# Zachary-Luk/3D-Denoising-Diffusion-Model

Hardware: AMD Instinct MI355X
Metric: denoised 64³ volumes/sec @250 DDPM steps, 1/2/4/8 MI355X; PSNR vs ref (higher is better)
Workload: dtype f32 (conv products: 3x f16-split MFMA, f32 accumulate)

## Files before the change

3d-denoising-diffusion-model_amd/csrc/api.hip:

```cpp
#include <hip/hip_runtime.h>
#include <stdarg.h>
#include <stdio.h>
#include <string.h>
#include "conv3d_params.h"
#include "ddpm3d.h"
#include "ops.h"
#include "noise.h"

static thread_local char g_err[512] = "";

static int fail(int code, const char* fmt, ...) {
    va_list ap;
    va_start(ap, fmt);
    vsnprintf(g_err, sizeof(g_err), fmt, ap);
    va_end(ap);
    return code;
}
static int launched(hipError_t e, const char* what) {
    if (e == hipSuccess) return DDPM3D_OK;
    return fail(DDPM3D_ELAUNCH, "%s: %s", what, hipGetErrorString(e));
}

extern "C" {

// ... 188 lines not shown
        route = ddpm3d_pw_ok(k, c, d->ksize) ? ROUTE_PW : ROUTE_GENERAL;
    return DDPM3D_OK;
}

int ddpm3d_conv3d(const ddpm3d_conv_desc* d, void* stream) {
    ConvK k;
    ConvCfg c;
    int route = ROUTE_GENERAL;
    const int ok = conv_prepare(d, k, c, route, true);
    if (ok != DDPM3D_OK) return ok;
    if (route == ROUTE_SKINNY)
        return launched(ddpm3d_launch_conv_skinny(k, d->precision, (hipStream_t)stream), "conv3d (skinny)");
    const int rc = route == ROUTE_PW ? launched(ddpm3d_launch_conv_pw(k, c, (hipStream_t)stream), "conv3d (1x1)")
                                     : launched(ddpm3d_launch_conv(k, c, (hipStream_t)stream), "conv3d");
    if (rc != DDPM3D_OK || c.S == 1) return rc;
    return launched(ddpm3d_launch_splitk_reduce(k, (hipStream_t)stream), "conv3d split-K reduce");
}

static int base_prec(int p) {
    return p == DDPM3D_PREC_F16X3_WZ ? DDPM3D_PREC_F16X3 : p == DDPM3D_PREC_F16_WZ ? DDPM3D_PREC_F16
         : p == DDPM3D_PREC_BF16_WZ ? DDPM3D_PREC_BF16 : p;
}
static int skip_prepare(const ddpm3d_conv_desc* d, const ddpm3d_conv_skip* sk, ddpm3d_conv_desc& sd, ConvK& k, ConvCfg& c,
                        bool& fused, bool for_launch) {
    fused = false;
    if (!d || !sk) return fail(DDPM3D_EINVAL, "conv3d_skip: null descriptor");
    if (d->res_mode != DDPM3D_RES_NONE || d->res)
        return fail(DDPM3D_EINVAL, "conv3d_skip: conv2 carries no residual of its own (the skip conv is its residual)");
    if (d->out_layout != DDPM3D_OUT_NDHWC) return fail(DDPM3D_EINVAL, "conv3d_skip: NDHWC output only");
    if (d->ksize != 3) return fail(DDPM3D_EINVAL, "conv3d_skip: conv2 is a 3x3x3 conv (ksize %d)", d->ksize);
// ... 32 lines not shown
    k.sk_bound = sk->in_bound; k.sk_bound_count = sk->in_bound_count; k.sk_bound_stride = sk->in_bound_stride;
    k.sk_blocks_per_split = (sd.Cin / 32 + c.S - 1) / c.S;
    return DDPM3D_OK;
}

int ddpm3d_conv3d_skip(const ddpm3d_conv_desc* d, const ddpm3d_conv_skip* sk, void* stream) {
    ddpm3d_conv_desc sd;
    ConvK k;
    ConvCfg c;
    bool fused = false;
    const int ok = skip_prepare(d, sk, sd, k, c, fused, true);
    if (ok != DDPM3D_OK) return ok;
    if (fused) {
        const int rc = launched(ddpm3d_launch_conv(k, c, (hipStream_t)stream), "conv3d_skip");
        if (rc != DDPM3D_OK || c.S == 1) return rc;
        return launched(ddpm3d_launch_splitk_reduce(k, (hipStream_t)stream), "conv3d_skip split-K reduce");
    }
    const int rc = ddpm3d_conv3d(&sd, stream);
    if (rc != DDPM3D_OK) return rc;
    ddpm3d_conv_desc d2 = *d;
    d2.res = d->out;
    d2.res_mode = DDPM3D_RES_SAME;
    if (d->io_dtype & DDPM3D_IO_OUT_BF16) d2.io_dtype |= DDPM3D_IO_RES_BF16;
    return ddpm3d_conv3d(&d2, stream);
}

int ddpm3d_conv_skip_fused(const ddpm3d_conv_desc* d, const ddpm3d_conv_skip* sk) {
    ddpm3d_conv_desc sd;
    ConvK k;
    ConvCfg c;
// ... 1017 lines not shown
```

3d-denoising-diffusion-model_amd/csrc/conv3d.hip:

```cpp
#include <hip/hip_runtime.h>
#include "conv3d_load.h"
#include "conv3d_epilogue.h"

template <int PREC, int PIPEM, int KS, int WN, int MT, int TXL, int TYL>
__global__ __launch_bounds__(256, (PIPEM == 2 ? 1 : (TXL == 2 ? 2 : 3))) void conv3d_kernel(const ConvK p) {
    constexpr int CK = DDPM3D_CONV_CK;
    constexpr int PIPE = PIPEM == 1 ? 1 : 0;
    constexpr int SXY = PIPEM == 2 ? 2 : 1;
    constexpr int WM = 4 / WN;
    constexpr int TX = 1 << TXL, TY = 1 << TYL;
    constexpr int TZ = WM * MT * 32 / (TX * TY);
    constexpr int PAD = KS / 2;
    constexpr int HX = SXY * (TX - 1) + KS, HY = SXY * (TY - 1) + KS, HZ = TZ + 2 * PAD;
    constexpr int HV = HX * HY * HZ;
    constexpr int VS = 5;
    constexpr int RY = LdsGeom<TX, HX, HY>::RY;
    constexpr int RZ = LdsGeom<TX, HX, HY>::RZ;
    constexpr int QPV = CK / 4;
    constexpr int NT = KS * KS * KS;
    constexpr int NL = (HV * QPV + 255) / 256;

    extern __shared__ __attribute__((aligned(16))) unsigned char lds[];

    const int tid = threadIdx.x;
// ... 367 lines not shown

#if DDPM3D_PREC_ONLY == 3
#include "conv3d_wz.h"
#ifndef DDPM3D_WZ_T84
#define DDPM3D_WZ_T84 1
#endif
hipError_t ddpm3d_launch_conv_wz(const ConvK& k, const ConvCfg& c, hipStream_t st) {
    const int gy = k.CoutPad / 128;
    const int gx = k.N * k.tilesZ * k.tilesY * k.tilesX;
#ifdef DDPM3D_WZ_STAMPS
    constexpr size_t stamp_lds = 4 * WZ_NSTAMP * 8;
#else
    constexpr size_t stamp_lds = 0;
#endif
    constexpr size_t lds = (size_t)WzGeom::BUF + stamp_lds;
    if (k.sk_w != nullptr) {
        if (c.PREC != DDPM3D_PREC_F16X3_WZ) return hipErrorInvalidValue;
        constexpr size_t slds4 = (size_t)WzGeomT<4>::BUF + stamp_lds, slds84 = (size_t)WzGeomT<8, 4>::BUF + stamp_lds;
        if (c.TXL == 2)
            hipLaunchKernelGGL((conv3d_wz_kernel<WZ_F16X3_SKIP, 4, 4>), dim3(gx, gy, k.ksplit), dim3(256), slds4, st, k);
        else if (DDPM3D_WZ_T84 && k.H % 8 == 0 && k.D % 4 == 0) {
            ConvK k2 = k;
            k2.tilesY = 2 * k.tilesY;
            k2.tilesZ = k.tilesZ / 2;
            hipLaunchKernelGGL((conv3d_wz_kernel<WZ_F16X3_SKIP, 4, 8, 4>), dim3(gx, gy, k.ksplit), dim3(256), slds84, st, k2);
        } else
            hipLaunchKernelGGL((conv3d_wz_kernel<WZ_F16X3_SKIP, 4>), dim3(gx, gy, k.ksplit), dim3(256), lds, st, k);
        return hipGetLastError();
    }
    if (k.hint & DDPM3D_HINT_UP_PHASE) {
// ... 96 lines not shown
```

3d-denoising-diffusion-model_amd/csrc/conv3d_params.h:

```cpp
#pragma once
#include <hip/hip_runtime.h>
#include <stddef.h>
#include <stdlib.h>
#include "ddpm3d.h"

#define DDPM3D_CONV_CK 16
#define DDPM3D_REDUCE_VOX 16
#define DDPM3D_X3_W_TARGET 8.0f

struct ConvK {
    const float* src0;
    const float* src1;
    const float* affA;
    const float* affB;
    const float* w;
    const float* bias;
    const float* res;
    float* out;
    double* stats;
    float* partial;
    const float* wscale;
    const float* in_bound;
    int in_bound_count, in_bound_stride;
    unsigned w_bytes, src0_bytes, src1_bytes;
// ... 106 lines not shown
    }
    const long long vox = (long long)D * H * W;
    c.reduce_vox = DDPM3D_REDUCE_VOX;
    while (c.reduce_vox > 4 &&
           (long long)N * ((vox + c.reduce_vox - 1) / c.reduce_vox) * ((Cout / 4 + 63) / 64) < 1024)
        c.reduce_vox /= 2;
    ddpm3d_conv_cfg_split(c, best, N, D, H, W, Cout);
    return c;
}

static inline bool ddpm3d_skip_fuse_rule(int N, int D, int H, int W, int Cx, int Cout, const ConvCfg& c) {
    (void)N; (void)D; (void)H; (void)W; (void)Cx; (void)Cout; (void)c;
    return true;
}

static inline size_t ddpm3d_packed_bytes(int Cout, int Cin, int ksize, int prec) {
    const size_t taps = (prec == DDPM3D_PREC_F16X3_WZ || prec == DDPM3D_PREC_F16_WZ || prec == DDPM3D_PREC_BF16_WZ)
                            ? 36 : (size_t)ksize * ksize * ksize;
    const size_t body = taps * ddpm3d_cin_pad(Cin) * ddpm3d_cout_pad(Cout) * 4;
    return prec != 0 ? body + (size_t)ddpm3d_cout_pad(Cout) * 4 : body;
}

static inline size_t ddpm3d_up_phase_body_bytes(int Cout, int Cin) {
    return (size_t)64 * ddpm3d_cin_pad(Cin) * ddpm3d_cout_pad(Cout) * 4;
}
static inline size_t ddpm3d_up_phase_bytes(int Cout, int Cin) {
    return ddpm3d_packed_bytes(Cout, Cin, 3, DDPM3D_PREC_F16X3_WZ) + ddpm3d_up_phase_body_bytes(Cout, Cin) +
           (size_t)ddpm3d_cout_pad(Cout) * 4;
}
struct UpPhaseGeom { int TX, TY, tilesX, tilesY, tilesZ; };
// ... 101 lines not shown
```

3d-denoising-diffusion-model_amd/csrc/conv3d_stage.h:

```cpp
#pragma once
#include "conv3d_epilogue.h"

enum { WZ_F16X3 = 0, WZ_F16 = 1, WZ_BF16 = 2,
       WZ_F16X3_UP = 3,
       WZ_F16X3_SKIP = 4 };

__device__ __forceinline__ void split_pair(float s0, float s1, unsigned& hi, unsigned& lo) {
    float l0, l1;
    asm("v_cvt_pk_f16_f32 %0, %3, %4\n\t"
        "v_fma_mix_f32 %1, %0, -1.0, %3 op_sel:[0,0,0] op_sel_hi:[1,0,0]\n\t"
        "v_fma_mix_f32 %2, %0, -1.0, %4 op_sel:[1,0,0] op_sel_hi:[1,0,0]"
        : "=&v"(hi), "=&v"(l0), "=&v"(l1)
        : "v"(s0), "v"(s1));
    asm("v_cvt_pk_f16_f32 %0, %1, %2" : "=v"(lo) : "v"(l0), "v"(l1));
}

template <int TX_, int TY_ = TX_>
struct WzGeomT {
    static constexpr int CK = DDPM3D_CONV_CK;
    static constexpr int TX = TX_, TY = TY_, HX = TX_ + 2, HY = TY_ + 2, NP = 4, VS = 5;
    static constexpr int RP = TX_ * TY_;
    static constexpr int NZP = 64 / RP;
    static constexpr int NPL = 2 * NZP + 2;
    static constexpr int RY = LdsGeom<TX_, HX, HY>::RY;
// ... 179 lines not shown
```

3d-denoising-diffusion-model_amd/csrc/conv3d_wz.h:

```cpp
#pragma once
#include "conv3d_stage.h"

#ifdef DDPM3D_WZ_STAMPS
#define WZ_NSTAMP 48
#define WZ_STAMP(i) do { if (lane == 0) wz_stamps[(i)] = __builtin_amdgcn_s_memtime(); } while (0)
#else
#define WZ_STAMP(i) do { } while (0)
#endif

template <int MODE_, int IL = 0, int TX = 8, int TY = TX>
__global__ __launch_bounds__(256, 2) void conv3d_wz_kernel(const ConvK p) {
    constexpr bool PHASE = MODE_ == WZ_F16X3_UP;
    constexpr bool SKIP = MODE_ == WZ_F16X3_SKIP;
    constexpr int MODE = (PHASE || SKIP) ? (int)WZ_F16X3 : MODE_;
    typedef WzGeomT<TX, TY> G;
    constexpr bool X3 = MODE == WZ_F16X3;
    constexpr int CK = DDPM3D_CONV_CK, NT = PHASE ? 16 : 36;
    constexpr int TPJ = NT / 4;
    constexpr int TXL = TX == 8 ? 3 : 2, TYL = TY == 8 ? 3 : 2;
    constexpr int VS = G::VS, RY = G::RY, RZ = G::RZ;

    extern __shared__ __attribute__((aligned(16))) unsigned char lds[];

    const int tid = threadIdx.x;
    const int lane = tid & 63;
    const int wn = __builtin_amdgcn_readfirstlane(tid >> 6);
    const int half = lane >> 5;
#ifdef DDPM3D_WZ_STAMPS
    unsigned long long* wz_stamps = reinterpret_cast<unsigned long long*>(lds + G::BUF) + wn * WZ_NSTAMP;
    WZ_STAMP(0);
#endif

    const WgId wg = wg_id(p);
    int tile = wg.tile;
    const int tx_i = tile % p.tilesX; tile /= p.tilesX;
    const int ty_i = tile % p.tilesY; tile /= p.tilesY;
    const int tz_i = tile % p.tilesZ; tile /= p.tilesZ;
    const int ph = PHASE ? (tile & 3) : 0;
    const int py = ph >> 1, px = ph & 1;
    const int n = PHASE ? tile >> 2 : tile;
    const int x0 = tx_i * TX, y0 = ty_i * TY, z0 = tz_i * 2 * G::NZP;

    int arow[2];
#pragma unroll
    for (int t = 0; t < 2; ++t) {
        const int m = t * 32 + (lane & 31);
        const int pos = m % G::RP;
        arow[t] = (m / G::RP) * G::PAIR + ((pos >> TXL) * RY + (pos & (TX - 1)) * VS + half) * 16;
        if constexpr (PHASE) arow[t] += (py * RY + px * VS) * 16;
    }

    const int cout = wg.cy * 128 + wn * 32 + (lane & 31);
    const float pre_ws = cout < p.Cout ? p.wscale[cout] : 1.0f;
    const float pre_bias = cout < p.Cout ? p.bias[(size_t)n * p.bias_stride_n + cout] : 0.0f;
    const __amdgpu_buffer_rsrc_t wrsrc = make_rsrc(p.w, p.w_bytes);
    const unsigned wlane = ((unsigned)cout * 2 + half) * 16;
    const unsigned wpart = (unsigned)p.CoutPad * 32;
    const unsigned wchunk_stride = 2 * wpart;
    const unsigned wtap_stride = (unsigned)(p.CinPad / CK) * wchunk_stride;

    f32x16 acc[4][2];
#pragma unroll
    for (int j = 0; j < 4; ++j)
#pragma unroll
        for (int t = 0; t < 2; ++t)
#pragma unroll
            for (int i = 0; i < 16; ++i) acc[j][t][i] = 0.0f;

    const int nchunks = p.CinPad / CK;
    const int chunk_begin = wg.split * p.chunks_per_split;
    const int chunk_end = min(nchunks, chunk_begin + p.chunks_per_split);

    ActScale asc = {1.0f, 1.0f};
    float bound_raw = 0.0f;
    if constexpr (MODE != WZ_BF16) bound_raw = act_scale_load(p, n);
    float sk_bound_raw = 0.0f;
    ActScale ax = {1.0f, 1.0f};
    if constexpr (SKIP)
        if (lane < p.sk_bound_count) sk_bound_raw = p.sk_bound[((size_t)n * p.sk_bound_count + lane) * p.sk_bound_stride];
    StageLaneT<G> sl = stage_lane<G, PHASE>(p, tid, n, y0, x0, max(z0 - 1, 0), 1.0f);
    stage_zero_border(sl, lds, 1, tid);
    StageRawT<G> raw;
    if (chunk_begin < chunk_end) stage_issue(p, sl, raw, n, z0, chunk_begin);
    if constexpr (MODE != WZ_BF16) {
        asc = act_scale_finish(bound_raw, 2.0f);
        if constexpr (SKIP) ax = act_scale_finish(sk_bound_raw, 1.0f);
        stage_lane_scale(p, sl, asc.s);
    }
    WZ_STAMP(1);

    constexpr int L = X3 ? 1 : 0;
#ifndef DDPM3D_WZ_RING_X3
#define DDPM3D_WZ_RING_X3 4
#endif
#ifndef DDPM3D_WZ_RING_X1
// ... 92 lines not shown
#pragma unroll
                for (int i = 0; i < (X3 ? 2 : 1); ++i) {
                    __builtin_amdgcn_sched_group_barrier(0x008, 1, 0);
                    __builtin_amdgcn_sched_group_barrier(0x020, 1, 0);
                }
#pragma unroll
                for (int i = 0; i < (X3 ? 4 : 2); ++i) {
                    __builtin_amdgcn_sched_group_barrier(0x008, 1, 0);
                    __builtin_amdgcn_sched_group_barrier(0x100, 1, 0);
                }
            }
        }
        if constexpr (IL == 3 || IL == 4 || IL == 6) __builtin_amdgcn_s_setprio(0);
        WZ_STAMP(6 + (chunk - chunk_begin) * 5);
    }
    WZ_STAMP(42);

    f32x16 outv[4];
#pragma unroll
    for (int t = 0; t < 2; ++t) {
        outv[t] = acc[0][t] + acc[1][t] + acc[2][t];
        outv[2 + t] = acc[1][t] - acc[2][t] - acc[3][t];
    }
    const int tile_in_n = ((ph * p.tilesZ + tz_i) * p.tilesY + ty_i) * p.tilesX + tx_i;
    if constexpr (SKIP) {
        const int tid_ = tid;
        constexpr int XB = 32, XROW = VS * 16, XCH = 128 * XROW;
        static_assert(2 * XCH <= G::BUF, "an x block fits the tile's image");
        const int nxb = (p.sk_C0 + p.sk_C1) / XB;
        const int xb_begin = wg.split * p.sk_blocks_per_split;
        const int xb_end = min(nxb, xb_begin + p.sk_blocks_per_split);
        int tid = tid_;
        asm volatile("" : "+v"(tid));
        const int lane = tid & 63, half = lane >> 5;
        const int xq = tid & 7;
        unsigned xv0[4], xv1[4];
#pragma unroll
        for (int i = 0; i < 4; ++i) {
            const int m = (tid >> 3) + 32 * i;
            const int z = z0 + epi_tz<TXL, TYL, G::NZP != 1>(m), y = y0 + ((m >> TXL) & (TY - 1)), x = x0 + (m & (TX - 1));
            const bool inb = z < p.D && y < p.H && x < p.W;
            const unsigned vox = (unsigned)(((n * p.D + z) * p.H + y) * p.W + x);
            xv0[i] = inb ? (vox * (unsigned)p.sk_C0 + xq * 4u) * 4u : DDPM3D_OOB_OFFSET;
            xv1[i] = inb ? (vox * (unsigned)p.sk_C1 + xq * 4u) * 4u : DDPM3D_OOB_OFFSET;
        }
        const int xl = ((xq >> 2) * 128 + (tid >> 3)) * XROW + (xq & 3) * 8;
        const int xa = ((lane & 31) * VS + half) * 16;
        auto x_issue = [&](const int b, u32x4 (&xr)[4]) {
            const bool valid = b < xb_end;
            const int c0 = b * XB;
            const bool from0 = c0 < p.sk_C0;
            const __amdgpu_buffer_rsrc_t rs = make_rsrc(from0 ? p.sk_src0 : p.sk_src1,
                                                        valid ? (from0 ? p.sk_src0_bytes : p.sk_src1_bytes) : 0u);
            const unsigned soff = valid ? (unsigned)(from0 ? c0 : c0 - p.sk_C0) * 4u : 0u;
#pragma unroll
            for (int i = 0; i < 4; ++i) xr[i] = buffer_load16(rs, from0 ? xv0[i] : xv1[i], soff);
        };
        auto w_issue = [&](const int b, u32x4 (&wq)[2][2]) {
            const bool valid = b < xb_end;
            const __amdgpu_buffer_rsrc_t rs = make_rsrc(p.sk_w, valid ? p.sk_w_bytes : 0u);
            const unsigned soff = valid ? (unsigned)(2 * b) * wchunk_stride : 0u;
#pragma unroll
// ... 33 lines not shown
                const h8 bhi = __builtin_bit_cast(h8, wq[c][0]), blo = __builtin_bit_cast(h8, wq[c][1]);
#pragma unroll
                for (int u = 0; u < 4; ++u) {
                    const unsigned char* a = lds + c * XCH + u * 32 * XROW + xa;
                    const h8 ahi = *reinterpret_cast<const h8*>(a), alo = *reinterpret_cast<const h8*>(a + 32);
                    outv[u] = mfma16<false>(alo, bhi, outv[u]);
                    outv[u] = mfma16<false>(ahi, blo, outv[u]);
                    outv[u] = mfma16<false>(ahi, bhi, outv[u]);
                }
            }
        };
        for (int b = xb_begin; b < xb_end; b += 2) {
            x_block(b, xr, wa, wb);
            x_block(b + 1, xr, wb, wa);
        }
        const float bias2 = pre_bias + sk_bias;
        if (p.ksplit > 1)
            conv_epilogue<1, 1, 4, TXL, TYL, true, G::NZP != 1, true, false>(p, outv, n, z0, y0, x0, tile_in_n, 0, cout, half, wg.split,
                                                                     ax.inv, true, sk_ws, bias2, 0, 0);
        else
            conv_epilogue<1, 1, 4, TXL, TYL, false, G::NZP != 1, false, false>(p, outv, n, z0, y0, x0, tile_in_n, 0, cout, half, wg.split,
                                                                     ax.inv, true, sk_ws, bias2, 0, 0);
        return;
    }
    #ifndef DDPM3D_WZ_WIDE_X3
#define DDPM3D_WZ_WIDE_X3 0
#endif
#ifndef DDPM3D_WZ_LEAN
#define DDPM3D_WZ_LEAN 1
#endif
    constexpr bool LEAN = DDPM3D_WZ_LEAN && MODE != WZ_F16X3;
    const float ws1[1] = {pre_ws}, bs1[1] = {pre_bias};
    if (p.ksplit > 1) {
        if (LEAN && conv_epilogue_lean<1, 1, 4, 1, TXL, TYL, G::NZP != 1, true>(p, outv, n, z0, y0, x0, tile_in_n, 0, cout, half,
                                                                                         wg.split, asc.inv, ws1, bs1)) {
        } else
        conv_epilogue<1, 1, 4, TXL, TYL, true, G::NZP != 1, true, PHASE>(p, outv, n, z0, y0, x0, tile_in_n, 0, cout, half, wg.split,
                                                                 asc.inv, true, pre_ws, pre_bias, py, px);
    } else if (LEAN &&
               conv_epilogue_lean<1, 1, 4, 1, TXL, TYL, G::NZP != 1, false>(p, outv, n, z0, y0, x0, tile_in_n, 0, cout, half, wg.split,
                                                                           asc.inv, ws1, bs1)) {
    } else
    conv_epilogue<1, 1, 4, TXL, TYL, MODE != WZ_F16X3 || DDPM3D_WZ_WIDE_X3, G::NZP != 1, false, PHASE>(p, outv, n, z0, y0, x0, tile_in_n, 0, cout, half, wg.split,
                                                                 asc.inv, true, pre_ws, pre_bias, py, px);
#ifdef DDPM3D_WZ_STAMPS
    WZ_STAMP(43);
    if (lane == 0) {
        wz_stamps[44] = __builtin_amdgcn_s_getreg((31 << 11) | 4);
        wz_stamps[45] = __builtin_amdgcn_s_getreg((31 << 11) | 20);
        wz_stamps[46] = __builtin_amdgcn_s_memrealtime();
    }
    if (p.partial != nullptr && lane < WZ_NSTAMP) {
        const size_t wgl = blockIdx.x + (size_t)gridDim.x * (blockIdx.y + (size_t)gridDim.y * blockIdx.z);
        float* dump = p.partial + (p.ksplit > 1 ? (size_t)p.ksplit * p.N * p.D * p.H * p.W * p.Cout : (size_t)0);
        reinterpret_cast<unsigned long long*>(dump)[(wgl * 4 + wn) * WZ_NSTAMP + lane] = wz_stamps[lane];
    }
#endif
}
```

3d-denoising-diffusion-model_amd/csrc/unet_plan.hip:

```cpp
#include <hip/hip_runtime.h>
#include <stdarg.h>
#include <stdio.h>
#include <string.h>
#include <map>
#include <new>
#include <vector>
#include "ddpm3d.h"

namespace {

struct Act {
    size_t off = 0;
    int C = 0, D = 0, H = 0, W = 0;
    int esize = 4;
    size_t stats_off = 0;
    int rows = 0;
    size_t bytes(int N) const { return (size_t)N * D * H * W * C * esize; }
    long long voxels() const { return (long long)D * H * W; }
};

enum StepKind { S_CONV, S_FINALIZE, S_ABSMAX, S_PAD, S_POOL, S_ATTN };

struct Step {
    int kind;
// ... 87 lines not shown
        int act = DDPM3D_ACT_NONE, in_mode = DDPM3D_IN_SAME;
        const Act* res = nullptr; int res_mode = DDPM3D_RES_NONE;
        bool planar = false, want_stats = true, bias_per_n = false;
        bool ncdhw_out = false;
        size_t bound = 0; int bound_first = 0, bound_count = 0, bound_stride = 0; bool has_bound = false;
        int film_off = 0;
        const ddpm3d_conv_weights* skip_w = nullptr;
        const Act* x0 = nullptr; const Act* x1 = nullptr;
        size_t xbound = 0; int xbound_first = 0; bool has_xbound = false;
        bool* fused = nullptr;
    };
    bool conv_step(const ddpm3d_conv_weights& pc, ConvArgs a, int* step_index = nullptr) {
        ddpm3d_conv_desc d;
        memset(&d, 0, sizeof(d));
        const bool wz = pc.w_packed_wz && !a.planar && (a.in_mode == DDPM3D_IN_SAME || a.in_mode == DDPM3D_IN_UP);
        d.precision = wz ? (pc.precision_wz & ~DDPM3D_WZ_UP_PHASE_IMAGE) : (pc.precision & ~DDPM3D_SKIP_TWO_CALLS);
        d.w_packed = wz ? pc.w_packed_wz : pc.w_packed;
        if (wz && (pc.precision_wz & DDPM3D_WZ_UP_PHASE_IMAGE) && a.in_mode == DDPM3D_IN_UP)
            d.kernel_hint = DDPM3D_HINT_UP_PHASE;
        d.bias = pc.bias;
        d.Cout = pc.Cout; d.ksize = pc.ksize;
        const Act* geo = a.out ? a.out : a.src0;
        d.N = N; d.D = geo->D; d.H = geo->H; d.W = geo->W;
        d.out_layout = a.ncdhw_out ? DDPM3D_OUT_NCDHW : DDPM3D_OUT_NDHWC;
        if (a.planar) {
            d.in_mode = DDPM3D_IN_PLANAR2; d.Cin = 2; d.C0 = 1; d.C1 = 1;
        } else {
            d.in_mode = a.in_mode;
            d.src0 = (const float*)at(a.src0->off); d.C0 = a.src0->C;
            if (a.src1) { d.src1 = (const float*)at(a.src1->off); d.C1 = a.src1->C; }
            d.Cin = d.C0 + d.C1;
            if (d.Cin != pc.Cin) return fail("conv %dx%d fed %d channels", pc.Cout, pc.Cin, d.Cin);
            if (a.src0->esize == 2) d.io_dtype |= DDPM3D_IO_SRC0_BF16;
            if (a.src1 && a.src1->esize == 2) d.io_dtype |= DDPM3D_IO_SRC1_BF16;
// ... 370 lines not shown
```

3d-denoising-diffusion-model_amd/guided_diffusion/_hip.py:

```python

import ctypes as C
import os

import torch

_HERE = os.path.dirname(os.path.abspath(__file__))
LIB_PATH = os.environ.get("DDPM3D_LIB") or os.path.normpath(os.path.join(_HERE, "..", "csrc", "libddpm3d.so"))

IN_SAME, IN_POOL, IN_UP, IN_PLANAR2, IN_STRIDE2 = 0, 1, 2, 3, 4
RES_NONE, RES_SAME, RES_POOL, RES_UP = 0, 1, 2, 3
ACT_NONE, ACT_SILU = 0, 1
OUT_NDHWC, OUT_NCDHW = 0, 1
F_LEARN_SIGMA, F_PREDICT_XSTART, F_CLIP = 1, 2, 4
NCOEF = 8
NQCOEF = 4
NSCOEF = 8
S_CX, S_W0, S_W1, S_W2, S_CZ = 0, 1, 2, 3, 4
PREC_F32, PREC_F16X3, PREC_F16, PREC_F16X3_WZ, PREC_F16_WZ, PREC_BF16, PREC_BF16_WZ = 0, 1, 2, 3, 4, 5, 6
PRECISIONS = {"f32": PREC_F32, "f16x3": PREC_F16X3, "f16": PREC_F16, "bf16": PREC_BF16}
WINOGRAD_OF = {PREC_F16X3: PREC_F16X3_WZ, PREC_F16: PREC_F16_WZ, PREC_BF16: PREC_BF16_WZ}
IO_SRC0_BF16, IO_SRC1_BF16, IO_OUT_BF16, IO_RES_BF16 = 1, 2, 4, 8
IO_HALF_IS_F16 = 16
ABI_VERSION = 13
MAX_DRAWS = 64
MAX_QUANTILES = 8
HINT_WSTAT_OFF, HINT_WSTAT_ON = 0x100, 0x200
HINT_SPLITK_SHIFT = 16
HINT_WZ_ORDER_SHIFT = 12
HINT_UP_PHASE = 0x400
WZ_UP_PHASE_IMAGE = 0x100
SKIP_TWO_CALLS = 0x100

_fp = C.c_void_p


class ConvDesc(C.Structure):
    _fields_ = [
        ("N", C.c_int32), ("D", C.c_int32), ("H", C.c_int32), ("W", C.c_int32),
        ("Cin", C.c_int32), ("Cout", C.c_int32), ("ksize", C.c_int32), ("in_mode", C.c_int32),
        ("src0", _fp), ("src1", _fp), ("C0", C.c_int32), ("C1", C.c_int32),
        ("aff_a", _fp), ("aff_b", _fp), ("act", C.c_int32), ("precision", C.c_int32),
        ("w_packed", _fp), ("bias", _fp), ("bias_stride_n", C.c_int32), ("res_mode", C.c_int32),
        ("res", _fp), ("out", _fp), ("out_layout", C.c_int32), ("stats_rows", C.c_int32),
        ("stats", _fp), ("workspace", _fp), ("workspace_bytes", C.c_size_t),
# ... 251 lines not shown
```

3d-denoising-diffusion-model_amd/guided_diffusion/engine.py:

```python

import collections
import ctypes as C
import math
import os

import torch

from . import _hip as H


class Act:
    __slots__ = ("buf", "C", "D", "H", "W", "stats", "rows")

    def __init__(self, buf, Cn, D, Hh, W, stats, rows):
        self.buf, self.C, self.D, self.H, self.W, self.stats, self.rows = buf, Cn, D, Hh, W, stats, rows

    @property
    def half(self):
        return self.buf.dtype in (torch.bfloat16, torch.float16)

    @property
    def voxels(self):
        return self.D * self.H * self.W

# ... 58 lines not shown
        qkv_perm = {}
        if getattr(topo, "new_attention_order", False):
            for e in topo.all_layers():
                if e.kind == "attn":
                    Cn, ch = e.cin, e.cin // e.heads
                    leg = torch.arange(3 * Cn)
                    h, part, i = leg // (3 * ch), (leg // ch) % 3, leg % ch
                    qkv_perm[e.prefix + ".qkv"] = (part * Cn + h * ch + i).to(device)
        params = dict(params)
        for base, perm in qkv_perm.items():
            params[base + ".weight"] = params[base + ".weight"][perm].contiguous()
            params[base + ".bias"] = params[base + ".bias"][perm].contiguous()
        self.p = params
        self.up_phase = (winograd and precision == "f16x3" and os.environ.get("DDPM3D_UP_PHASE", "1") != "0")
        self.skip_fuse = os.environ.get("DDPM3D_SKIP_FUSE", "1") != "0"
        up_conv1 = {e.prefix + ".in_layers.2" for e in topo.all_layers() if e.kind == "res" and e.updown == "up"}
        for name, t in params.items():
            if name.endswith(".weight") and t.dim() >= 3:
                base = name[:-len(".weight")]
                if t.dim() == 5:
                    w = t
                elif t.dim() == 4 and t.shape[2] == 3:
                    w = torch.zeros(t.shape[0], t.shape[1], 3, 3, 3, dtype=t.dtype, device=t.device)
                    w[:, :, 1] = t
                else:
                    w = t.reshape(t.shape[0], t.shape[1], 1, 1, 1)
                if base == first and not planar and w.shape[1] != self.cin_pad:
                    wp = torch.zeros(w.shape[0], self.cin_pad, *w.shape[2:], dtype=w.dtype, device=w.device)
                    wp[:, :w.shape[1]] = w
                    w = wp
# ... 57 lines not shown
            pl = _Plan(self, N, D, Hh, W)
            self.plans[key] = pl
        else:
            self.plans.move_to_end(key)
        return pl

    def _conv_weights(self, pc):
        w = H.ConvWeights()
        if pc is not None:
            w.w_packed, w.bias = H.ptr(pc.w), H.ptr(pc.b)
            w.Cout, w.Cin, w.ksize, w.precision = pc.Cout, pc.Cin, pc.k, pc.precision
            if pc.wz is not None:
                w.w_packed_wz, w.precision_wz = H.ptr(pc.wz.w), pc.wz.precision
                if pc.wz.up_phase:
                    w.precision_wz |= H.WZ_UP_PHASE_IMAGE
        return w

    def native_desc(self):
        if self._native_desc is not None:
            return self._native_desc[0]
        topo, p = self.topo, self.p
        layers, keep = [], []

        def one(e):
            L = H.Layer()
            L.updown, L.heads = H.UPDOWN[e.updown], e.heads
            if e.kind == "res":
                L.kind = H.LAYER_RES
                L.film_off = self.film_off[e.prefix]
                L.norm1_gamma, L.norm1_beta = H.ptr(p[e.prefix + ".in_layers.0.weight"]), H.ptr(p[e.prefix + ".in_layers.0.bias"])
# ... 333 lines not shown
            io |= H.IO_SRC1_BF16 if (len(srcs) > 1 and srcs[1].half) else 0
        io |= H.IO_OUT_BF16 if (out is not None and out.half) else 0
        io |= H.IO_RES_BF16 if (res is not None and res.half) else 0
        if io and self.half_dtype == torch.float16:
            io |= H.IO_HALF_IS_F16
        d.io_dtype = io
        if self.scaled:
            if bound is None or bound[0] is None:
                raise RuntimeError("conv_step without an input bound")
            d.in_bound = bound[0].data_ptr() + 4 * bound[1]
            d.in_bound_count, d.in_bound_stride = bound[2], bound[3]
        d.precision = pc_use.precision
        d.w_packed, d.bias = H.ptr(pc_use.w), H.ptr(pc.b)
        if pc_use.up_phase and in_mode == H.IN_UP:
            d.kernel_hint = H.HINT_UP_PHASE
        d.bias_stride_n = 0
        d.res_mode = res_mode
        if res is not None and res.C != pc.Cout:
            raise RuntimeError("residual has %d channels, the conv writes %d" % (res.C, pc.Cout))
        d.res = H.ptr(res.buf) if res is not None else 0
        sk = None
        if skip is not None:
            spc, xs, xb = skip
            sk = H.ConvSkip()
            sk.src0, sk.C0 = H.ptr(xs[0].buf), xs[0].C
            if len(xs) > 1:
                sk.src1, sk.C1 = H.ptr(xs[1].buf), xs[1].C
            sk.w_packed, sk.bias = H.ptr(spc.w), H.ptr(spc.b)
            sk.io_dtype = (H.IO_SRC0_BF16 if xs[0].half else 0) | (H.IO_SRC1_BF16 if len(xs) > 1 and xs[1].half else 0)
            if self.scaled:
# ... 169 lines not shown
```

include/ddpm3d.h:

```cpp
#ifndef DDPM3D_H
#define DDPM3D_H

#include <stddef.h>
#include <stdint.h>

#ifdef __cplusplus
extern "C" {
#endif

#define DDPM3D_ABI_VERSION 13

enum {
    DDPM3D_OK = 0,
    DDPM3D_EINVAL = -1,
    DDPM3D_ELAUNCH = -2,
    DDPM3D_ENOSUP = -3,
    DDPM3D_E2BIG = -4
};

enum {
    DDPM3D_IN_SAME = 0,
    DDPM3D_IN_POOL = 1,
    DDPM3D_IN_UP = 2,
    DDPM3D_IN_PLANAR2 = 3,
// ... 44 lines not shown
enum {
    DDPM3D_IO_SRC0_BF16 = 1,
    DDPM3D_IO_SRC1_BF16 = 2,
    DDPM3D_IO_OUT_BF16 = 4,
    DDPM3D_IO_RES_BF16 = 8,
    DDPM3D_IO_HALF_IS_F16 = 16
};

enum {
    DDPM3D_HINT_WSTAT_OFF = 0x100,
    DDPM3D_HINT_WSTAT_ON = 0x200,
    DDPM3D_HINT_WZ_ORDER_SHIFT = 12,
    DDPM3D_HINT_WZ_ORDER_MASK = 0x7000,
    DDPM3D_HINT_SPLITK_SHIFT = 16,
    DDPM3D_HINT_SPLITK_MASK = 0x3F0000,
    DDPM3D_HINT_UP_PHASE = 0x400
};

#define DDPM3D_WZ_UP_PHASE_IMAGE 0x100
#define DDPM3D_SKIP_TWO_CALLS 0x100

int ddpm3d_abi_version(void);
const char* ddpm3d_last_error(void);

enum {
    DDPM3D_PREC_F32 = 0,
    DDPM3D_PREC_F16X3 = 1,
    DDPM3D_PREC_F16 = 2,
    DDPM3D_PREC_F16X3_WZ = 3,
    DDPM3D_PREC_F16_WZ = 4,
    DDPM3D_PREC_BF16 = 5,
    DDPM3D_PREC_BF16_WZ = 6
};

// ... 355 lines not shown
```

Baseline: 0.3413.

## Pair split-K slices into one 512-thread workgroup with in-LDS partial sum

For f16x3 Winograd-z 3x3x3 convs that use split-K, two adjacent K slices now run as the two halves of one 512-thread workgroup. Each half has its own LDS image, and the halves add their accumulators through LDS before the epilogue. This halves the number of split-K slabs that are written to global memory and read back by the reduce kernel, which cuts partial-sum traffic. In exchange it doubles LDS per workgroup, adds barrier-matching padding loops for halves with uneven chunk counts, and lowers the number of resident workgroups.

```diff
diff --git a/3d-denoising-diffusion-model_amd/csrc/api.hip b/3d-denoising-diffusion-model_amd/csrc/api.hip
--- a/3d-denoising-diffusion-model_amd/csrc/api.hip
+++ b/3d-denoising-diffusion-model_amd/csrc/api.hip
@@ -226,6 +226,7 @@
     const int rc = route == ROUTE_PW ? launched(ddpm3d_launch_conv_pw(k, c, (hipStream_t)stream), "conv3d (1x1)")
                                      : launched(ddpm3d_launch_conv(k, c, (hipStream_t)stream), "conv3d");
     if (rc != DDPM3D_OK || c.S == 1) return rc;
+    if (route == ROUTE_GENERAL && ddpm3d_pair_launch(k, c)) k.ksplit = ddpm3d_pair_slabs(c.S);
     return launched(ddpm3d_launch_splitk_reduce(k, (hipStream_t)stream), "conv3d split-K reduce");
 }
 
@@ -288,6 +289,7 @@
     if (fused) {
         const int rc = launched(ddpm3d_launch_conv(k, c, (hipStream_t)stream), "conv3d_skip");
         if (rc != DDPM3D_OK || c.S == 1) return rc;
+        if (ddpm3d_pair_launch(k, c)) k.ksplit = ddpm3d_pair_slabs(c.S);
         return launched(ddpm3d_launch_splitk_reduce(k, (hipStream_t)stream), "conv3d_skip split-K reduce");
     }
     const int rc = ddpm3d_conv3d(&sd, stream);
diff --git a/3d-denoising-diffusion-model_amd/csrc/conv3d.hip b/3d-denoising-diffusion-model_amd/csrc/conv3d.hip
--- a/3d-denoising-diffusion-model_amd/csrc/conv3d.hip
+++ b/3d-denoising-diffusion-model_amd/csrc/conv3d.hip
@@ -405,6 +405,29 @@
     constexpr size_t stamp_lds = 0;
 #endif
     constexpr size_t lds = (size_t)WzGeom::BUF + stamp_lds;
+    if (ddpm3d_pair_launch(k, c)) {
+        const bool skip = k.sk_w != nullptr;
+        const dim3 grid(gx, gy, ddpm3d_pair_slabs(k.ksplit));
+        static DynLdsOnce once[4] = {};
+        const void* kern;
+        size_t plds;
+        ConvK k2 = k;
+        if (c.TXL == 2) {
+            kern = skip ? reinterpret_cast<const void*>(&conv3d_wz_kernel<WZ_F16X3_SKIP_PAIR, 4, 4, 4>)
+                        : reinterpret_cast<const void*>(&conv3d_wz_kernel<WZ_F16X3_PAIR, 4, 4, 4>);
+            plds = 2 * (size_t)WzGeomT<4>::BUF + 2 * stamp_lds;
+        } else {
+            kern = skip ? reinterpret_cast<const void*>(&conv3d_wz_kernel<WZ_F16X3_SKIP_PAIR, 4, 8, 4>)
+                        : reinterpret_cast<const void*>(&conv3d_wz_kernel<WZ_F16X3_PAIR, 4, 8, 4>);
+            plds = 2 * (size_t)WzGeomT<8, 4>::BUF + 2 * stamp_lds;
+            k2.tilesY = 2 * k.tilesY;
+            k2.tilesZ = k.tilesZ / 2;
+        }
+        const hipError_t attr = ddpm3d_allow_dynamic_lds(once[(c.TXL == 2 ? 0 : 2) + (skip ? 1 : 0)], kern, (int)plds);
+        if (attr != hipSuccess) return attr;
+        void* args[] = {&k2};
+        return hipLaunchKernel(kern, grid, dim3(512), args, plds, st);
+    }
     if (k.sk_w != nullptr) {
         if (c.PREC != DDPM3D_PREC_F16X3_WZ) return hipErrorInvalidValue;
         constexpr size_t slds4 = (size_t)WzGeomT<4>::BUF + stamp_lds, slds84 = (size_t)WzGeomT<8, 4>::BUF + stamp_lds;
diff --git a/3d-denoising-diffusion-model_amd/csrc/conv3d_params.h b/3d-denoising-diffusion-model_amd/csrc/conv3d_params.h
--- a/3d-denoising-diffusion-model_amd/csrc/conv3d_params.h
+++ b/3d-denoising-diffusion-model_amd/csrc/conv3d_params.h
@@ -144,6 +144,22 @@
     return true;
 }
 
+static inline bool ddpm3d_pair_split_rule(int N, int D, int H, int W, int Cin, int Cout, const ConvCfg& c) {
+    (void)D; (void)H; (void)W;
+    const long long blocks = (long long)N * c.tilesZ * c.tilesY * c.tilesX * (ddpm3d_cout_pad(Cout) / 128);
+    if (c.S <= 1 || blocks * c.S != 512) return false;
+    if (c.TXL == 2) return true;
+    return c.S == 4 && ddpm3d_cin_pad(Cin) / DDPM3D_CONV_CK <= 16;
+}
+static inline int ddpm3d_pair_slabs(int S) { return (S + 1) / 2; }
+static inline bool ddpm3d_pair_launch(const ConvK& k, const ConvCfg& c) {
+    if (c.PREC != DDPM3D_PREC_F16X3_WZ || c.KS != 3 || k.ksplit <= 1) return false;
+    if (k.hint & (DDPM3D_HINT_UP_PHASE | DDPM3D_HINT_WZ_ORDER_MASK | DDPM3D_HINT_PAIR_OFF)) return false;
+    if (!(c.TXL == 2 || (k.H % 8 == 0 && k.D % 4 == 0))) return false;
+    if (k.hint & DDPM3D_HINT_PAIR_ON) return true;
+    return ddpm3d_pair_split_rule(k.N, k.D, k.H, k.W, k.Cin, k.Cout, c);
+}
+
 static inline size_t ddpm3d_packed_bytes(int Cout, int Cin, int ksize, int prec) {
     const size_t taps = (prec == DDPM3D_PREC_F16X3_WZ || prec == DDPM3D_PREC_F16_WZ || prec == DDPM3D_PREC_BF16_WZ)
                             ? 36 : (size_t)ksize * ksize * ksize;
diff --git a/3d-denoising-diffusion-model_amd/csrc/conv3d_stage.h b/3d-denoising-diffusion-model_amd/csrc/conv3d_stage.h
--- a/3d-denoising-diffusion-model_amd/csrc/conv3d_stage.h
+++ b/3d-denoising-diffusion-model_amd/csrc/conv3d_stage.h
@@ -3,7 +3,9 @@
 
 enum { WZ_F16X3 = 0, WZ_F16 = 1, WZ_BF16 = 2,
        WZ_F16X3_UP = 3,
-       WZ_F16X3_SKIP = 4 };
+       WZ_F16X3_SKIP = 4,
+       WZ_F16X3_PAIR = 5,
+       WZ_F16X3_SKIP_PAIR = 6 };
 
 __device__ __forceinline__ void split_pair(float s0, float s1, unsigned& hi, unsigned& lo) {
     float l0, l1;
diff --git a/3d-denoising-diffusion-model_amd/csrc/conv3d_wz.h b/3d-denoising-diffusion-model_amd/csrc/conv3d_wz.h
--- a/3d-denoising-diffusion-model_amd/csrc/conv3d_wz.h
+++ b/3d-denoising-diffusion-model_amd/csrc/conv3d_wz.h
@@ -9,10 +9,11 @@
 #endif
 
 template <int MODE_, int IL = 0, int TX = 8, int TY = TX>
-__global__ __launch_bounds__(256, 2) void conv3d_wz_kernel(const ConvK p) {
+__global__ __launch_bounds__((MODE_ == WZ_F16X3_PAIR || MODE_ == WZ_F16X3_SKIP_PAIR) ? 512 : 256, 2) void conv3d_wz_kernel(const ConvK p) {
+    constexpr bool PAIR = MODE_ == WZ_F16X3_PAIR || MODE_ == WZ_F16X3_SKIP_PAIR;
     constexpr bool PHASE = MODE_ == WZ_F16X3_UP;
-    constexpr bool SKIP = MODE_ == WZ_F16X3_SKIP;
-    constexpr int MODE = (PHASE || SKIP) ? (int)WZ_F16X3 : MODE_;
+    constexpr bool SKIP = MODE_ == WZ_F16X3_SKIP || MODE_ == WZ_F16X3_SKIP_PAIR;
+    constexpr int MODE = (PHASE || SKIP || PAIR) ? (int)WZ_F16X3 : MODE_;
     typedef WzGeomT<TX, TY> G;
     constexpr bool X3 = MODE == WZ_F16X3;
     constexpr int CK = DDPM3D_CONV_CK, NT = PHASE ? 16 : 36;
@@ -22,16 +23,21 @@
 
     extern __shared__ __attribute__((aligned(16))) unsigned char lds[];
 
-    const int tid = threadIdx.x;
+    static_assert(!PAIR || (X3 && !PHASE), "the paired form: f16x3 and its SKIP form");
+    static_assert(!PAIR || 2 * G::BUF >= 256 * 64 * 4, "the upper half's outv fit the two images");
+    const int tid = PAIR ? (int)(threadIdx.x & 255) : (int)threadIdx.x;
     const int lane = tid & 63;
     const int wn = __builtin_amdgcn_readfirstlane(tid >> 6);
     const int half = lane >> 5;
+    const int kh = PAIR ? __builtin_amdgcn_readfirstlane((int)(threadIdx.x >> 8)) : 0;
+    const int hoff = kh * G::BUF;
 #ifdef DDPM3D_WZ_STAMPS
-    unsigned long long* wz_stamps = reinterpret_cast<unsigned long long*>(lds + G::BUF) + wn * WZ_NSTAMP;
+    unsigned long long* wz_stamps = reinterpret_cast<unsigned long long*>(lds + (PAIR ? 2 : 1) * G::BUF) + (kh * 4 + wn) * WZ_NSTAMP;
     WZ_STAMP(0);
 #endif
 
     const WgId wg = wg_id(p);
+    const int split = PAIR ? 2 * wg.split + kh : wg.split;
     int tile = wg.tile;
     const int tx_i = tile % p.tilesX; tile /= p.tilesX;
     const int ty_i = tile % p.tilesY; tile /= p.tilesY;
@@ -47,6 +53,7 @@
         const int m = t * 32 + (lane & 31);
         const int pos = m % G::RP;
         arow[t] = (m / G::RP) * G::PAIR + ((pos >> TXL) * RY + (pos & (TX - 1)) * VS + half) * 16;
+        if constexpr (PAIR) arow[t] += hoff;
         if constexpr (PHASE) arow[t] += (py * RY + px * VS) * 16;
     }
 
@@ -68,7 +75,7 @@
             for (int i = 0; i < 16; ++i) acc[j][t][i] = 0.0f;
 
     const int nchunks = p.CinPad / CK;
-    const int chunk_begin = wg.split * p.chunks_per_split;
+    const int chunk_begin = split * p.chunks_per_split;
     const int chunk_end = min(nchunks, chunk_begin + p.chunks_per_split);
 
     ActScale asc = {1.0f, 1.0f};
@@ -79,6 +86,10 @@
     if constexpr (SKIP)
         if (lane < p.sk_bound_count) sk_bound_raw = p.sk_bound[((size_t)n * p.sk_bound_count + lane) * p.sk_bound_stride];
     StageLaneT<G> sl = stage_lane<G, PHASE>(p, tid, n, y0, x0, max(z0 - 1, 0), 1.0f);
+    if constexpr (PAIR) {
+#pragma unroll
+        for (int i = 0; i < G::NL; ++i) sl.lds[i] += hoff;
+    }
     stage_zero_border(sl, lds, 1, tid);
     StageRawT<G> raw;
     if (chunk_begin < chunk_end) stage_issue(p, sl, raw, n, z0, chunk_begin);
@@ -201,7 +212,57 @@
         if constexpr (IL == 3 || IL == 4 || IL == 6) __builtin_amdgcn_s_setprio(0);
         WZ_STAMP(6 + (chunk - chunk_begin) * 5);
     }
+    if constexpr (PAIR) {
+        const int lo_begin = 2 * wg.split * p.chunks_per_split;
+        const int lo_n = max(0, min(nchunks, lo_begin + p.chunks_per_split) - lo_begin);
+        for (int i = max(0, chunk_end - chunk_begin); i < lo_n; ++i) {
+            __syncthreads();
+            __syncthreads();
+        }
+    }
     WZ_STAMP(42);
+#ifdef DDPM3D_WZ_STAMPS
+    auto stamps_dump = [&]() {
+        if (lane == 0) {
+            wz_stamps[44] = __builtin_amdgcn_s_getreg((31 << 11) | 4);
+            wz_stamps[45] = __builtin_amdgcn_s_getreg((31 << 11) | 20);
+            wz_stamps[46] = __builtin_amdgcn_s_memrealtime();
+        }
+        if (p.partial != nullptr && lane < WZ_NSTAMP) {
+            const size_t wgl = blockIdx.x + (size_t)gridDim.x * (blockIdx.y + (size_t)gridDim.y * blockIdx.z);
+            float* dump = p.partial + (p.ksplit > 1 ? (size_t)p.ksplit * p.N * p.D * p.H * p.W * p.Cout : (size_t)0);
+            reinterpret_cast<unsigned long long*>(dump)[((wgl * (PAIR ? 2 : 1) + kh) * 4 + wn) * WZ_NSTAMP + lane] = wz_stamps[lane];
+        }
+    };
+#endif
+    f32x16 outh[2];
+    auto pair_sum = [&](const f32x16 (&o)[4]) {
+        if constexpr (PAIR) {
+            WZ_STAMP(40);
+            __syncthreads();
+            f32x4* ex = reinterpret_cast<f32x4*>(lds) + tid;
+            const int snd = kh ? 2 : 0, rcv = kh ? 0 : 2;
+#pragma unroll
+            for (int t = 0; t < 2; ++t)
+#pragma unroll
+                for (int g = 0; g < 4; ++g) {
+                    f32x4 q;
+#pragma unroll
+                    for (int i = 0; i < 4; ++i) q[i] = kh ? o[t][4 * g + i] : o[2 + t][4 * g + i];
+                    ex[((snd + t) * 4 + g) * 256] = q;
+                }
+            __syncthreads();
+#pragma unroll
+            for (int t = 0; t < 2; ++t)
+#pragma unroll
+                for (int g = 0; g < 4; ++g) {
+                    const f32x4 q = ex[((rcv + t) * 4 + g) * 256];
+#pragma unroll
+                    for (int i = 0; i < 4; ++i) outh[t][4 * g + i] = (kh ? o[2 + t][4 * g + i] : o[t][4 * g + i]) + q[i];
+                }
+            WZ_STAMP(41);
+        }
+    };
 
     f32x16 outv[4];
 #pragma unroll
@@ -215,7 +276,7 @@
         constexpr int XB = 32, XROW = VS * 16, XCH = 128 * XROW;
         static_assert(2 * XCH <= G::BUF, "an x block fits the tile's image");
         const int nxb = (p.sk_C0 + p.sk_C1) / XB;
-        const int xb_begin = wg.split * p.sk_blocks_per_split;
+        const int xb_begin = split * p.sk_blocks_per_split;
         const int xb_end = min(nxb, xb_begin + p.sk_blocks_per_split);
         int tid = tid_;
         asm volatile("" : "+v"(tid));
@@ -231,8 +292,8 @@
             xv0[i] = inb ? (vox * (unsigned)p.sk_C0 + xq * 4u) * 4u : DDPM3D_OOB_OFFSET;
             xv1[i] = inb ? (vox * (unsigned)p.sk_C1 + xq * 4u) * 4u : DDPM3D_OOB_OFFSET;
         }
-        const int xl = ((xq >> 2) * 128 + (tid >> 3)) * XROW + (xq & 3) * 8;
-        const int xa = ((lane & 31) * VS + half) * 16;
+        const int xl = ((xq >> 2) * 128 + (tid >> 3)) * XROW + (xq & 3) * 8 + hoff;
+        const int xa = ((lane & 31) * VS + half) * 16 + hoff;
         auto x_issue = [&](const int b, u32x4 (&xr)[4]) {
             const bool valid = b < xb_end;
             const int c0 = b * XB;
@@ -296,8 +357,23 @@
             x_block(b, xr, wa, wb);
             x_block(b + 1, xr, wb, wa);
         }
+        if constexpr (PAIR) {
+            const int lo_b = 2 * wg.split * p.sk_blocks_per_split;
+            const int lo_turns = (max(0, min(nxb, lo_b + p.sk_blocks_per_split) - lo_b) + 1) / 2;
+            for (int i = (max(0, xb_end - xb_begin) + 1) / 2; i < lo_turns; ++i) {
+                __syncthreads(); __syncthreads(); __syncthreads(); __syncthreads();
+            }
+        }
+        pair_sum(outv);
         const float bias2 = pre_bias + sk_bias;
-        if (p.ksplit > 1)
+        if constexpr (PAIR) {
+            if (kh)
+                conv_epilogue<1, 2, 2, TXL, TYL, true, G::NZP != 1, true, false>(p, outh, n, z0, y0, x0, tile_in_n, 1, cout, half, wg.split,
+                                                                         ax.inv, true, sk_ws, bias2, 0, 0);
+            else
+                conv_epilogue<1, 2, 2, TXL, TYL, true, G::NZP != 1, true, false>(p, outh, n, z0, y0, x0, tile_in_n, 0, cout, half, wg.split,
+                                                                         ax.inv, true, sk_ws, bias2, 0, 0);
+        } else if (p.ksplit > 1)
             conv_epilogue<1, 1, 4, TXL, TYL, true, G::NZP != 1, true, false>(p, outv, n, z0, y0, x0, tile_in_n, 0, cout, half, wg.split,
                                                                      ax.inv, true, sk_ws, bias2, 0, 0);
         else
@@ -313,7 +389,15 @@
 #endif
     constexpr bool LEAN = DDPM3D_WZ_LEAN && MODE != WZ_F16X3;
     const float ws1[1] = {pre_ws}, bs1[1] = {pre_bias};
-    if (p.ksplit > 1) {
+    pair_sum(outv);
+    if constexpr (PAIR) {
+        if (kh)
+            conv_epilogue<1, 2, 2, TXL, TYL, true, G::NZP != 1, true, false>(p, outh, n, z0, y0, x0, tile_in_n, 1, cout, half, wg.split,
+                                                                     asc.inv, true, pre_ws, pre_bias, 0, 0);
+        else
+            conv_epilogue<1, 2, 2, TXL, TYL, true, G::NZP != 1, true, false>(p, outh, n, z0, y0, x0, tile_in_n, 0, cout, half, wg.split,
+                                                                     asc.inv, true, pre_ws, pre_bias, 0, 0);
+    } else if (p.ksplit > 1) {
         if (LEAN && conv_epilogue_lean<1, 1, 4, 1, TXL, TYL, G::NZP != 1, true>(p, outv, n, z0, y0, x0, tile_in_n, 0, cout, half,
                                                                                          wg.split, asc.inv, ws1, bs1)) {
         } else
@@ -327,15 +411,6 @@
                                                                  asc.inv, true, pre_ws, pre_bias, py, px);
 #ifdef DDPM3D_WZ_STAMPS
     WZ_STAMP(43);
-    if (lane == 0) {
-        wz_stamps[44] = __builtin_amdgcn_s_getreg((31 << 11) | 4);
-        wz_stamps[45] = __builtin_amdgcn_s_getreg((31 << 11) | 20);
-        wz_stamps[46] = __builtin_amdgcn_s_memrealtime();
-    }
-    if (p.partial != nullptr && lane < WZ_NSTAMP) {
-        const size_t wgl = blockIdx.x + (size_t)gridDim.x * (blockIdx.y + (size_t)gridDim.y * blockIdx.z);
-        float* dump = p.partial + (p.ksplit > 1 ? (size_t)p.ksplit * p.N * p.D * p.H * p.W * p.Cout : (size_t)0);
-        reinterpret_cast<unsigned long long*>(dump)[(wgl * 4 + wn) * WZ_NSTAMP + lane] = wz_stamps[lane];
-    }
+    stamps_dump();
 #endif
 }
diff --git a/3d-denoising-diffusion-model_amd/csrc/unet_plan.hip b/3d-denoising-diffusion-model_amd/csrc/unet_plan.hip
--- a/3d-denoising-diffusion-model_amd/csrc/unet_plan.hip
+++ b/3d-denoising-diffusion-model_amd/csrc/unet_plan.hip
@@ -125,10 +125,11 @@
         ddpm3d_conv_desc d;
         memset(&d, 0, sizeof(d));
         const bool wz = pc.w_packed_wz && !a.planar && (a.in_mode == DDPM3D_IN_SAME || a.in_mode == DDPM3D_IN_UP);
-        d.precision = wz ? (pc.precision_wz & ~DDPM3D_WZ_UP_PHASE_IMAGE) : (pc.precision & ~DDPM3D_SKIP_TWO_CALLS);
+        d.precision = wz ? (pc.precision_wz & ~(DDPM3D_WZ_UP_PHASE_IMAGE | DDPM3D_WZ_PAIR_OFF)) : (pc.precision & ~DDPM3D_SKIP_TWO_CALLS);
         d.w_packed = wz ? pc.w_packed_wz : pc.w_packed;
         if (wz && (pc.precision_wz & DDPM3D_WZ_UP_PHASE_IMAGE) && a.in_mode == DDPM3D_IN_UP)
             d.kernel_hint = DDPM3D_HINT_UP_PHASE;
+        if (wz && (pc.precision_wz & DDPM3D_WZ_PAIR_OFF)) d.kernel_hint |= DDPM3D_HINT_PAIR_OFF;
         d.bias = pc.bias;
         d.Cout = pc.Cout; d.ksize = pc.ksize;
         const Act* geo = a.out ? a.out : a.src0;
diff --git a/3d-denoising-diffusion-model_amd/guided_diffusion/_hip.py b/3d-denoising-diffusion-model_amd/guided_diffusion/_hip.py
--- a/3d-denoising-diffusion-model_amd/guided_diffusion/_hip.py
+++ b/3d-denoising-diffusion-model_amd/guided_diffusion/_hip.py
@@ -28,6 +28,8 @@
 HINT_SPLITK_SHIFT = 16
 HINT_WZ_ORDER_SHIFT = 12
 HINT_UP_PHASE = 0x400
+HINT_PAIR_OFF, HINT_PAIR_ON = 0x800, 0x8000
+WZ_PAIR_OFF = 0x200
 WZ_UP_PHASE_IMAGE = 0x100
 SKIP_TWO_CALLS = 0x100
 
diff --git a/3d-denoising-diffusion-model_amd/guided_diffusion/engine.py b/3d-denoising-diffusion-model_amd/guided_diffusion/engine.py
--- a/3d-denoising-diffusion-model_amd/guided_diffusion/engine.py
+++ b/3d-denoising-diffusion-model_amd/guided_diffusion/engine.py
@@ -96,6 +96,7 @@
         self.p = params
         self.up_phase = (winograd and precision == "f16x3" and os.environ.get("DDPM3D_UP_PHASE", "1") != "0")
         self.skip_fuse = os.environ.get("DDPM3D_SKIP_FUSE", "1") != "0"
+        self.pair_split = os.environ.get("DDPM3D_PAIR_SPLIT", "1") != "0"
         up_conv1 = {e.prefix + ".in_layers.2" for e in topo.all_layers() if e.kind == "res" and e.updown == "up"}
         for name, t in params.items():
             if name.endswith(".weight") and t.dim() >= 3:
@@ -183,6 +184,8 @@
                 w.w_packed_wz, w.precision_wz = H.ptr(pc.wz.w), pc.wz.precision
                 if pc.wz.up_phase:
                     w.precision_wz |= H.WZ_UP_PHASE_IMAGE
+                if not self.pair_split:
+                    w.precision_wz |= H.WZ_PAIR_OFF
         return w
 
     def native_desc(self):
@@ -546,6 +549,8 @@
         d.w_packed, d.bias = H.ptr(pc_use.w), H.ptr(pc.b)
         if pc_use.up_phase and in_mode == H.IN_UP:
             d.kernel_hint = H.HINT_UP_PHASE
+        if pc_use is pc.wz and not self.eng.pair_split:
+            d.kernel_hint |= H.HINT_PAIR_OFF
         d.bias_stride_n = 0
         d.res_mode = res_mode
         if res is not None and res.C != pc.Cout:
diff --git a/include/ddpm3d.h b/include/ddpm3d.h
--- a/include/ddpm3d.h
+++ b/include/ddpm3d.h
@@ -82,10 +82,13 @@
     DDPM3D_HINT_WZ_ORDER_MASK = 0x7000,
     DDPM3D_HINT_SPLITK_SHIFT = 16,
     DDPM3D_HINT_SPLITK_MASK = 0x3F0000,
-    DDPM3D_HINT_UP_PHASE = 0x400
+    DDPM3D_HINT_UP_PHASE = 0x400,
+    DDPM3D_HINT_PAIR_OFF = 0x800,
+    DDPM3D_HINT_PAIR_ON = 0x8000
 };
 
 #define DDPM3D_WZ_UP_PHASE_IMAGE 0x100
+#define DDPM3D_WZ_PAIR_OFF 0x200
 #define DDPM3D_SKIP_TWO_CALLS 0x100
 
 int ddpm3d_abi_version(void);
```

New measurement: 0.3414, median of 3. About the same (+0.0%).
